# westlake-repl/Adapter4Rec

Measured on NVIDIA B200. Metric: train user-sequences/s (SASRec + BERT-base LoRA r=8 adapter-tuning step: fwd+bwd+allreduce+Adam), higher is better.
Workload: dtype bf16

## Files before the change

adapter4rec_b200/csrc/attention_small.cu:

```cuda
#include "a4r_common.cuh"
#include "mma_sync.cuh"

namespace {

constexpr int LP = 32;
constexpr int WARPS_PER_CTA = 4;

struct AttnParams {
  const __nv_bfloat16* qkv;
  __nv_bfloat16* out;
  const __nv_bfloat16* dout;
  const void* mask;
  int64_t ld_qkv, ld_out, mask_ld;
  int N, L, heads;
  int mask_dtype;
  const int32_t* cu_seqlens;
  int causal;
  float scale, mask_neg;
  uint32_t drop_thr16;
  float drop_scale;
  uint64_t drop_seed, drop_offset;
};

A4R_DEVICE void prob_dropout(float (&s)[2][4][4], const AttnParams& p, int n, int h, int lane) {
  const int g = lane >> 2, t = lane & 3;
  const uint64_t base = p.drop_offset + (static_cast<uint64_t>(n) * p.heads + h) * (32 * 8);
  const uint64_t seed = rng_seed(p.drop_seed);
#pragma unroll
  for (int mt = 0; mt < 2; ++mt)
#pragma unroll
    for (int hh = 0; hh < 2; ++hh) {
      const int i = mt * 16 + hh * 8 + g;
#pragma unroll
      for (int np = 0; np < 2; ++np) {
        const uint64_t r = rng64(seed, base + static_cast<uint64_t>(i) * 8 + np * 4 + t);
#pragma unroll
        for (int q = 0; q < 2; ++q)
#pragma unroll
          for (int e = 0; e < 2; ++e) {
            float& x = s[mt][np * 2 + q][hh * 2 + e];
            x = rng_keep(r, q * 2 + e, p.drop_thr16) ? x * p.drop_scale : 0.0f;
          }
      }
    }
}

template <int COLS>
struct Tile {
  static constexpr int kChunks = COLS / 8;
  static constexpr int kBytes = LP * COLS * 2;
  A4R_DEVICE static uint32_t off(int row, int chunk) {
    const int x = COLS == 64 ? row : (row >> 1);
    return static_cast<uint32_t>(row * COLS * 2 + (((chunk ^ x) & (kChunks - 1)) << 4));
  }
};

template <int COLS>
A4R_DEVICE void load_a(uint32_t (&a)[4], uint32_t base, int m0, int k0, int lane) {
  const int mi = lane >> 3, r = lane & 7;
  const int row = m0 + r + ((mi & 1) << 3);
  const int chunk = (k0 >> 3) + (mi >> 1);
  ldsm_x4(a, base + Tile<COLS>::off(row, chunk));
}
template <int COLS>
A4R_DEVICE void load_a_t(uint32_t (&a)[4], uint32_t base, int m0, int k0, int lane) {
  const int mi = lane >> 3, r = lane & 7;
  const int row = k0 + r + ((mi >> 1) << 3);
  const int chunk = (m0 >> 3) + (mi & 1);
  ldsm_x4_t(a, base + Tile<COLS>::off(row, chunk));
}
template <int COLS>
A4R_DEVICE void load_b_nk(uint32_t (&b)[4], uint32_t base, int n0, int k0, int lane) {
  const int mi = lane >> 3, r = lane & 7;
  const int row = n0 + r + ((mi >> 1) << 3);
  const int chunk = (k0 >> 3) + (mi & 1);
  ldsm_x4(b, base + Tile<COLS>::off(row, chunk));
}
template <int COLS>
A4R_DEVICE void load_b_kn(uint32_t (&b)[4], uint32_t base, int n0, int k0, int lane) {
  const int mi = lane >> 3, r = lane & 7;
  const int row = k0 + r + ((mi & 1) << 3);
  const int chunk = (n0 >> 3) + (mi >> 1);
  ldsm_x4_t(b, base + Tile<COLS>::off(row, chunk));
}

template <int DH>
A4R_DEVICE void load_tile(uint8_t* tile, const __nv_bfloat16* g, int64_t ld, int L, int lane) {
  constexpr int CH = DH / 8;
  const uint32_t base = smem_u32(tile);
#pragma unroll
  for (int i = lane; i < LP * CH; i += 32) {
    const int row = i / CH, ch = i % CH;
    const bool ok = row < L;
    const __nv_bfloat16* src = g + (ok ? static_cast<int64_t>(row) * ld + ch * 8 : 0);
    const int sz = ok ? 16 : 0;
    asm volatile("cp.async.cg.shared.global [%0], [%1], 16, %2;" ::"r"(base + Tile<DH>::off(row, ch)), "l"(src), "r"(sz)
                 : "memory");
// ... 101 lines not shown
#pragma unroll
      for (int nt = 0; nt < 4; ++nt)
#pragma unroll
        for (int e = 0; e < 2; ++e) {
          const float ex = __expf(s[mt][nt][h * 2 + e] - mx);
          s[mt][nt][h * 2 + e] = ex;
          sum += ex;
        }
      sum += __shfl_xor_sync(0xffffffffu, sum, 1);
      sum += __shfl_xor_sync(0xffffffffu, sum, 2);
      const float inv = 1.0f / sum;
#pragma unroll
      for (int nt = 0; nt < 4; ++nt)
#pragma unroll
        for (int e = 0; e < 2; ++e) s[mt][nt][h * 2 + e] *= inv;
    }
  }
}

A4R_DEVICE uint32_t build_keymask(const AttnParams& p, const SeqSpan& sq, int lane) {
  const bool ok = lane < sq.L ? key_valid(p, sq, lane) : false;
  return __ballot_sync(0xffffffffu, ok);
}

A4R_DEVICE void acc_to_a(uint32_t (&a)[4], const float (&c0)[4], const float (&c1)[4]) {
  a[0] = pack_bf16x2(c0[0], c0[1]);
  a[1] = pack_bf16x2(c0[2], c0[3]);
  a[2] = pack_bf16x2(c1[0], c1[1]);
  a[3] = pack_bf16x2(c1[2], c1[3]);
}

template <int DH>
__global__ void __launch_bounds__(WARPS_PER_CTA * 32, 3) attn_fwd_kernel(const AttnParams p) {
  extern __shared__ __align__(128) uint8_t smem_attn[];
  constexpr int TB = Tile<DH>::kBytes;
  const int warp = threadIdx.x >> 5, lane = threadIdx.x & 31;
  uint8_t* my = smem_attn + warp * 3 * TB;
  const int64_t total = static_cast<int64_t>(p.N) * p.heads;
  for (int64_t w = static_cast<int64_t>(blockIdx.x) * WARPS_PER_CTA + warp; w < total;
       w += static_cast<int64_t>(gridDim.x) * WARPS_PER_CTA) {
    const int n = static_cast<int>(w / p.heads), h = static_cast<int>(w % p.heads);
    const int64_t Hd = static_cast<int64_t>(p.heads) * DH;
    const SeqSpan sq = seq_span(p, n);
    const __nv_bfloat16* q = p.qkv + sq.row0 * p.ld_qkv + h * DH;
    load_tile<DH>(my, q, p.ld_qkv, sq.L, lane);
    load_tile<DH>(my + TB, q + Hd, p.ld_qkv, sq.L, lane);
    load_tile<DH>(my + 2 * TB, q + 2 * Hd, p.ld_qkv, sq.L, lane);
    const uint32_t km = build_keymask(p, sq, lane);
    cp_async_wait_all();
    __syncwarp();
    const uint32_t sQ = smem_u32(my), sK = sQ + TB, sV = sK + TB;
    float s[2][4][4];
    scores_softmax<DH>(s, sQ, sK, p, sq.L, lane, km);
    if (p.drop_thr16 != 0) prob_dropout(s, p, n, h, lane);
    float o[2][DH / 8][4];
#pragma unroll
    for (int mt = 0; mt < 2; ++mt)
#pragma unroll
      for (int nt = 0; nt < DH / 8; ++nt)
#pragma unroll
        for (int e = 0; e < 4; ++e) o[mt][nt][e] = 0.0f;
#pragma unroll
    for (int ks = 0; ks < 2; ++ks) {
      uint32_t a0[4], a1[4];
      acc_to_a(a0, s[0][2 * ks], s[0][2 * ks + 1]);
      acc_to_a(a1, s[1][2 * ks], s[1][2 * ks + 1]);
#pragma unroll
      for (int np = 0; np < DH / 16; ++np) {
        uint32_t b[4];
        load_b_kn<DH>(b, sV, np * 16, ks * 16, lane);
        const uint32_t b0[2] = {b[0], b[1]}, b1[2] = {b[2], b[3]};
        mma_bf16_16816(o[0][np * 2], a0, b0);
        mma_bf16_16816(o[0][np * 2 + 1], a0, b1);
        mma_bf16_16816(o[1][np * 2], a1, b0);
        mma_bf16_16816(o[1][np * 2 + 1], a1, b1);
      }
    }
    __syncwarp();
    acc_to_tile<DH, DH / 8>(my, o, 1.f, 1.f, 1.f, 1.f, lane);
    __syncwarp();
    store_tile<DH>(my, p.out + sq.row0 * p.ld_out + h * DH, p.ld_out, sq.L, lane);
    __syncwarp();
  }
}

template <int DH>
__global__ void __launch_bounds__(WARPS_PER_CTA * 32) attn_bwd_kernel(const AttnParams p) {
  extern __shared__ __align__(128) uint8_t smem_attn[];
  constexpr int TB = Tile<DH>::kBytes;
  constexpr int PB = Tile<32>::kBytes;
  const int warp = threadIdx.x >> 5, lane = threadIdx.x & 31;
  uint8_t* my = smem_attn + warp * (4 * TB + 2 * PB);
  const int64_t total = static_cast<int64_t>(p.N) * p.heads;
  for (int64_t w = static_cast<int64_t>(blockIdx.x) * WARPS_PER_CTA + warp; w < total;
       w += static_cast<int64_t>(gridDim.x) * WARPS_PER_CTA) {
    const int n = static_cast<int>(w / p.heads), h = static_cast<int>(w % p.heads);
    const int64_t Hd = static_cast<int64_t>(p.heads) * DH;
    const SeqSpan sq = seq_span(p, n);
    const __nv_bfloat16* q = p.qkv + sq.row0 * p.ld_qkv + h * DH;
    uint8_t *tQ = my, *tK = my + TB, *tV = my + 2 * TB, *tdO = my + 3 * TB, *tP = my + 4 * TB, *tdS = tP + PB;
    load_tile<DH>(tQ, q, p.ld_qkv, sq.L, lane);
    load_tile<DH>(tK, q + Hd, p.ld_qkv, sq.L, lane);
    load_tile<DH>(tV, q + 2 * Hd, p.ld_qkv, sq.L, lane);
    load_tile<DH>(tdO, p.dout + sq.row0 * p.ld_out + h * DH, p.ld_out, sq.L, lane);
    const uint32_t km = build_keymask(p, sq, lane);
    cp_async_wait_all();
    __syncwarp();
    const uint32_t sQ = smem_u32(tQ), sK = smem_u32(tK), sV = smem_u32(tV), sdO = smem_u32(tdO), sP = smem_u32(tP),
                   sdS = smem_u32(tdS);
    float s[2][4][4];
    scores_softmax<DH>(s, sQ, sK, p, sq.L, lane, km);
    float dp[2][4][4];
#pragma unroll
    for (int mt = 0; mt < 2; ++mt)
#pragma unroll
      for (int nt = 0; nt < 4; ++nt)
#pragma unroll
        for (int e = 0; e < 4; ++e) dp[mt][nt][e] = 0.0f;
#pragma unroll
    for (int k0 = 0; k0 < DH; k0 += 16) {
      uint32_t a0[4], a1[4];
      load_a<DH>(a0, sdO, 0, k0, lane);
      load_a<DH>(a1, sdO, 16, k0, lane);
#pragma unroll
      for (int np = 0; np < 2; ++np) {
        uint32_t b[4];
        load_b_nk<DH>(b, sV, np * 16, k0, lane);
        const uint32_t b0[2] = {b[0], b[1]}, b1[2] = {b[2], b[3]};
        mma_bf16_16816(dp[0][np * 2], a0, b0);
        mma_bf16_16816(dp[0][np * 2 + 1], a0, b1);
        mma_bf16_16816(dp[1][np * 2], a1, b0);
        mma_bf16_16816(dp[1][np * 2 + 1], a1, b1);
      }
    }
    float sd[2][4][4];
#pragma unroll
    for (int mt = 0; mt < 2; ++mt)
#pragma unroll
      for (int nt = 0; nt < 4; ++nt)
#pragma unroll
        for (int e = 0; e < 4; ++e) sd[mt][nt][e] = s[mt][nt][e];
    if (p.drop_thr16 != 0) {
      prob_dropout(sd, p, n, h, lane);
#pragma unroll
      for (int mt = 0; mt < 2; ++mt)
#pragma unroll
        for (int nt = 0; nt < 4; ++nt)
#pragma unroll
          for (int e = 0; e < 4; ++e) dp[mt][nt][e] = (sd[mt][nt][e] != 0.0f) ? dp[mt][nt][e] * p.drop_scale : 0.0f;
    }
#pragma unroll
    for (int mt = 0; mt < 2; ++mt)
#pragma unroll
      for (int hh = 0; hh < 2; ++hh) {
        float d = 0.0f;
#pragma unroll
        for (int nt = 0; nt < 4; ++nt)
#pragma unroll
          for (int e = 0; e < 2; ++e) d += s[mt][nt][hh * 2 + e] * dp[mt][nt][hh * 2 + e];
        d += __shfl_xor_sync(0xffffffffu, d, 1);
        d += __shfl_xor_sync(0xffffffffu, d, 2);
#pragma unroll
        for (int nt = 0; nt < 4; ++nt)
#pragma unroll
          for (int e = 0; e < 2; ++e)
            dp[mt][nt][hh * 2 + e] = s[mt][nt][hh * 2 + e] * (dp[mt][nt][hh * 2 + e] - d) * p.scale;
      }
    acc_to_tile<32, 4>(tP, sd, 1.f, 1.f, 1.f, 1.f, lane);
    acc_to_tile<32, 4>(tdS, dp, 1.f, 1.f, 1.f, 1.f, lane);
    __syncwarp();
    float acc[2][DH / 8][4];
#pragma unroll
    for (int mt = 0; mt < 2; ++mt)
#pragma unroll
      for (int nt = 0; nt < DH / 8; ++nt)
#pragma unroll
        for (int e = 0; e < 4; ++e) acc[mt][nt][e] = 0.0f;
#pragma unroll
    for (int ks = 0; ks < 2; ++ks) {
      uint32_t a0[4], a1[4];
      acc_to_a(a0, dp[0][2 * ks], dp[0][2 * ks + 1]);
      acc_to_a(a1, dp[1][2 * ks], dp[1][2 * ks + 1]);
#pragma unroll
      for (int np = 0; np < DH / 16; ++np) {
        uint32_t b[4];
        load_b_kn<DH>(b, sK, np * 16, ks * 16, lane);
        const uint32_t b0[2] = {b[0], b[1]}, b1[2] = {b[2], b[3]};
        mma_bf16_16816(acc[0][np * 2], a0, b0);
        mma_bf16_16816(acc[0][np * 2 + 1], a0, b1);
        mma_bf16_16816(acc[1][np * 2], a1, b0);
        mma_bf16_16816(acc[1][np * 2 + 1], a1, b1);
      }
    }
    float dk[2][DH / 8][4], dv[2][DH / 8][4];
#pragma unroll
    for (int mt = 0; mt < 2; ++mt)
#pragma unroll
      for (int nt = 0; nt < DH / 8; ++nt)
#pragma unroll
        for (int e = 0; e < 4; ++e) dk[mt][nt][e] = dv[mt][nt][e] = 0.0f;
#pragma unroll
    for (int ks = 0; ks < 2; ++ks) {
      uint32_t a0[4], a1[4], p0[4], p1[4];
      load_a_t<32>(a0, sdS, 0, ks * 16, lane);
      load_a_t<32>(a1, sdS, 16, ks * 16, lane);
      load_a_t<32>(p0, sP, 0, ks * 16, lane);
      load_a_t<32>(p1, sP, 16, ks * 16, lane);
#pragma unroll
      for (int np = 0; np < DH / 16; ++np) {
        uint32_t b[4];
        load_b_kn<DH>(b, sQ, np * 16, ks * 16, lane);
        const uint32_t b0[2] = {b[0], b[1]}, b1[2] = {b[2], b[3]};
        mma_bf16_16816(dk[0][np * 2], a0, b0);
        mma_bf16_16816(dk[0][np * 2 + 1], a0, b1);
        mma_bf16_16816(dk[1][np * 2], a1, b0);
        mma_bf16_16816(dk[1][np * 2 + 1], a1, b1);
        uint32_t c[4];
        load_b_kn<DH>(c, sdO, np * 16, ks * 16, lane);
        const uint32_t c0[2] = {c[0], c[1]}, c1[2] = {c[2], c[3]};
        mma_bf16_16816(dv[0][np * 2], p0, c0);
        mma_bf16_16816(dv[0][np * 2 + 1], p0, c1);
        mma_bf16_16816(dv[1][np * 2], p1, c0);
        mma_bf16_16816(dv[1][np * 2 + 1], p1, c1);
      }
    }
    __syncwarp();
    acc_to_tile<DH, DH / 8>(tQ, acc, 1.f, 1.f, 1.f, 1.f, lane);
    acc_to_tile<DH, DH / 8>(tK, dk, 1.f, 1.f, 1.f, 1.f, lane);
    acc_to_tile<DH, DH / 8>(tV, dv, 1.f, 1.f, 1.f, 1.f, lane);
    __syncwarp();
    __nv_bfloat16* dq = p.out + sq.row0 * p.ld_qkv + h * DH;
    store_tile<DH>(tQ, dq, p.ld_qkv, sq.L, lane);
    store_tile<DH>(tK, dq + Hd, p.ld_qkv, sq.L, lane);
    store_tile<DH>(tV, dq + 2 * Hd, p.ld_qkv, sq.L, lane);
    __syncwarp();
  }
}

int check_common(const a4r_attn_args* a) {
  A4R_CHECK_ARG(a != nullptr, "attention: args is NULL");
  A4R_CHECK_ARG(a->qkv && a->out, "attention: qkv/out must be non-NULL");
  A4R_CHECK_ARG(a->L >= 1 && a->L <= LP, "attention_small: L must be in [1,32] (got %lld)", (long long)a->L);
  A4R_CHECK_ARG(a->head_dim == 32 || a->head_dim == 64, "attention_small: head_dim must be 32 or 64");
  A4R_CHECK_ARG(a->heads >= 1 && a->N >= 0, "attention: bad heads/N");
  A4R_CHECK_ARG(a->ld_qkv >= 3 * a->heads * a->head_dim && a->ld_qkv % 8 == 0, "attention: bad ld_qkv");
  A4R_CHECK_ARG(a->ld_out >= a->heads * a->head_dim && a->ld_out % 8 == 0, "attention: bad ld_out");
  A4R_CHECK_ARG(a4r_aligned16(a->qkv) && a4r_aligned16(a->out), "attention: pointers must be 16B aligned");
  A4R_CHECK_ARG(a->mask_dtype >= 0 && a->mask_dtype <= 2, "attention: mask_dtype must be 0,1,2");
  if (a->mask_dtype != 0)
    A4R_CHECK_ARG(a->mask != nullptr && (a->cu_seqlens != nullptr || a->mask_ld >= a->L), "attention: bad mask/mask_ld");
  A4R_CHECK_ARG(a->dropout_p >= 0.0f && a->dropout_p < 1.0f, "attention: dropout_p must be in [0,1)");
  return a4r_device_check();
}

AttnParams to_params(const a4r_attn_args* a) {
  AttnParams p;
  p.qkv = static_cast<const __nv_bfloat16*>(a->qkv);
  p.out = static_cast<__nv_bfloat16*>(a->out);
  p.dout = static_cast<const __nv_bfloat16*>(a->dout);
  p.mask = a->mask;
  p.ld_qkv = a->ld_qkv;
  p.ld_out = a->ld_out;
  p.mask_ld = a->mask_ld;
  p.N = static_cast<int>(a->N);
  p.L = static_cast<int>(a->L);
  p.cu_seqlens = a->cu_seqlens;
  p.heads = static_cast<int>(a->heads);
  p.mask_dtype = a->mask_dtype;
  p.causal = a->causal;
  p.scale = a->scale;
  p.mask_neg = a->mask_neg;
  p.drop_thr16 = static_cast<uint32_t>(a->dropout_p * 65536.0f + 0.5f);
  p.drop_scale = 65536.0f / static_cast<float>(65536u - p.drop_thr16);
  p.drop_seed = a->dropout_seed;
  p.drop_offset = a->dropout_offset;
  return p;
}

template <typename K>
int launch(K kernel, int smem, const AttnParams& p, cudaStream_t stream, bool* attr_done) {
  if (!*attr_done) {
    A4R_CUDA_OK(cudaFuncSetAttribute(kernel, cudaFuncAttributeMaxDynamicSharedMemorySize, smem));
    *attr_done = true;
  }
  const int64_t total = static_cast<int64_t>(p.N) * p.heads;
  int64_t blocks = (total + WARPS_PER_CTA - 1) / WARPS_PER_CTA;
  const int64_t cap = static_cast<int64_t>(a4r_num_sms()) * 8;
  if (blocks > cap) blocks = cap;
  kernel<<<static_cast<int>(blocks), WARPS_PER_CTA * 32, smem, stream>>>(p);
  A4R_LAUNCH_OK();
  a4r_count_launch(1);
  return A4R_OK;
}

}

extern "C" int a4r_attn_small_fwd(const a4r_attn_args* a, a4r_stream_t stream) {
  int rc = check_common(a);
  if (rc != A4R_OK) return rc;
  if (a->N == 0) return A4R_OK;
  const AttnParams p = to_params(a);
  static bool done64 = false, done32 = false;
  if (a->head_dim == 64)
    return launch(attn_fwd_kernel<64>, WARPS_PER_CTA * 3 * Tile<64>::kBytes, p, static_cast<cudaStream_t>(stream), &done64);
  return launch(attn_fwd_kernel<32>, WARPS_PER_CTA * 3 * Tile<32>::kBytes, p, static_cast<cudaStream_t>(stream), &done32);
}

extern "C" int a4r_attn_small_bwd(const a4r_attn_args* a, a4r_stream_t stream) {
  int rc = check_common(a);
  if (rc != A4R_OK) return rc;
  A4R_CHECK_ARG(a->dout != nullptr && a4r_aligned16(a->dout), "attention bwd: dout missing or unaligned");
  if (a->N == 0) return A4R_OK;
  const AttnParams p = to_params(a);
  static bool done64 = false, done32 = false;
  if (a->head_dim == 64)
    return launch(attn_bwd_kernel<64>, WARPS_PER_CTA * (4 * Tile<64>::kBytes + 2 * Tile<32>::kBytes), p,
                  static_cast<cudaStream_t>(stream), &done64);
  return launch(attn_bwd_kernel<32>, WARPS_PER_CTA * (4 * Tile<32>::kBytes + 2 * Tile<32>::kBytes), p,
                static_cast<cudaStream_t>(stream), &done32);
}
```

adapter4rec_b200/functional.py:

```python
import torch

from . import ops

BF16 = torch.bfloat16


PARAM_EPOCH = [0]


def bump_param_epoch():
    PARAM_EPOCH[0] += 1


class WeightCache:

    def __init__(self):
        self.key = None
        self.master = None
        self.w = None
        self.wt = None

    def get(self, weight, need_t=False):
        key = (weight.data_ptr(), weight._version, weight.device, PARAM_EPOCH[0] if weight.requires_grad else -1)
        if key != self.key:
# ... 230 lines not shown
        if cls.seed_address is not None:
            return cls.SEED_INDIRECT | int(cls.seed_address), off
        return cls.seed, off

    @classmethod
    def replay_seed(cls, step, base=None):
        z = ((cls.seed if base is None else int(base)) + 0x9E3779B97F4A7C15 * (int(step) + 1)) & 0xFFFFFFFFFFFFFFFF
        z = ((z ^ (z >> 30)) * 0xBF58476D1CE4E5B9) & 0xFFFFFFFFFFFFFFFF
        z = ((z ^ (z >> 27)) * 0x94D049BB133111EB) & 0xFFFFFFFFFFFFFFFF
        return (z ^ (z >> 31)) & 0x7FFFFFFFFFFFFFFF


class DropoutAddFunction(torch.autograd.Function):

    @staticmethod
    def forward(ctx, x, res, p):
        ctx.p = p
        ctx.rng = DropoutState.draw((x.numel() + 3) // 4)
        ctx.has_res = res is not None
        return ops.dropout(x.contiguous(), None if res is None else res.contiguous(), p, *ctx.rng)

    @staticmethod
    def backward(ctx, dy):
        dy = dy.contiguous()
        dx = ops.dropout(dy, None, ctx.p, *ctx.rng) if ctx.needs_input_grad[0] else None
        return dx, (dy if ctx.has_res and ctx.needs_input_grad[1] else None), None


def dropout_add(x, res, p):
    return DropoutAddFunction.apply(x, res, float(p))


class AddFunction(torch.autograd.Function):

    @staticmethod
    def forward(ctx, x, res):
        return ops.dropout(x.contiguous(), res.contiguous(), 0.0, 0, 0)

    @staticmethod
    def backward(ctx, dy):
        return (dy if ctx.needs_input_grad[0] else None), (dy if ctx.needs_input_grad[1] else None)


def add(x, res):
    return AddFunction.apply(x, res)


class AttentionFunction(torch.autograd.Function):
    @staticmethod
    def forward(ctx, qkv, mask, N, L, heads, head_dim, causal, mask_neg, dropout_p=0.0, scale=None, cu_seqlens=None):
        ctx.cfg = (N, L, heads, head_dim, causal, mask_neg, scale)
        ctx.cu = cu_seqlens
        ctx.mask = mask
        ctx.drop = None
        if dropout_p > 0.0:
            ctx.drop = (dropout_p,) + DropoutState.draw(N * heads * 32 * 8)
        out, lse = ops.attn_small_fwd(qkv, N, L, heads, head_dim, mask=mask, causal=causal, mask_neg=mask_neg, want_lse=True,
                                      dropout=ctx.drop, scale=scale, cu_seqlens=cu_seqlens)
        ctx.save_for_backward(qkv, lse, out if lse is not None else None)
        return out

    @staticmethod
    def backward(ctx, dctx):
        qkv, lse, out = ctx.saved_tensors
        N, L, heads, head_dim, causal, mask_neg, scale = ctx.cfg
        dqkv = ops.attn_small_bwd(qkv, dctx.contiguous(), N, L, heads, head_dim, mask=ctx.mask, causal=causal,
                                  mask_neg=mask_neg, lse=lse, ctx=out, dropout=ctx.drop, scale=scale, cu_seqlens=ctx.cu)
        return dqkv, None, None, None, None, None, None, None, None, None, None


def attention(qkv, mask, N, L, heads, head_dim, causal=False, mask_neg=ops.F32_MIN, dropout_p=0.0, scale=None,
              cu_seqlens=None):
    return AttentionFunction.apply(qkv, mask, N, L, heads, head_dim, causal, mask_neg, float(dropout_p), scale, cu_seqlens)


class GatherRowsFunction(torch.autograd.Function):

    @staticmethod
    def forward(ctx, x, idx):
        ctx.rows = x.shape[0]
        ctx.save_for_backward(idx)
        return ops.gather_rows(x.contiguous(), idx)

    @staticmethod
    def backward(ctx, dy):
        (idx,) = ctx.saved_tensors
        dx = torch.zeros((ctx.rows, dy.shape[1]), dtype=dy.dtype, device=dy.device)
        dx.index_copy_(0, idx, dy.contiguous())
        return dx, None


def gather_rows(x, idx):
    return GatherRowsFunction.apply(x, idx)


class ExpandRowsFunction(torch.autograd.Function):

    @staticmethod
    def forward(ctx, x, inverse, counts):
        ctx.save_for_backward(inverse, counts)
        return ops.gather_rows(x.contiguous(), inverse)

    @staticmethod
    def backward(ctx, dy):
        inverse, counts = ctx.saved_tensors
        order = torch.argsort(inverse, stable=True)
        grouped = dy.contiguous()[order].float()
        return torch.segment_reduce(grouped, "sum", lengths=counts, axis=0).to(dy.dtype), None, None


def expand_rows(x, inverse, counts):
    return ExpandRowsFunction.apply(x, inverse, counts)


_ROW_HASH = {}


def unique_rows(rows):
    N, W = rows.shape
    key = (rows.device, W)
# ... 404 lines not shown
```

adapter4rec_b200/lib.py:

```python
import ctypes
import os
from ctypes import POINTER, Structure, c_char_p, c_float, c_int32, c_int64, c_size_t, c_void_p

HERE = os.path.dirname(os.path.abspath(__file__))
LIB_PATH = os.path.join(HERE, "libadapter4rec_sm100.so")

A4R_OK, A4R_EINVAL, A4R_ECUDA, A4R_EARCH, A4R_EWORKSPACE = 0, -1, -2, -3, -4
EPI_LINEAR, EPI_GELU, EPI_RELU, EPI_DGELU, EPI_DRELU = 0, 1, 2, 3, 4


class GemmArgs(Structure):
    _fields_ = [
        ("A", c_void_p), ("lda", c_int64), ("B", c_void_p), ("ldb", c_int64),
        ("A2", c_void_p), ("lda2", c_int64), ("B2", c_void_p), ("ldb2", c_int64), ("K2", c_int64),
        ("C", c_void_p), ("ldc", c_int64), ("aux", c_void_p), ("ldaux", c_int64),
        ("residual", c_void_p), ("ldr", c_int64), ("residual2", c_void_p), ("ldr2", c_int64),
        ("bias", c_void_p), ("M", c_int64), ("N", c_int64), ("K", c_int64),
        ("alpha", c_float), ("epilogue", c_int32), ("out_f32", c_int32), ("block_n", c_int32),
        ("dropout_p", c_float), ("dropout_seed", ctypes.c_uint64), ("dropout_offset", ctypes.c_uint64),
        ("dropout_after_residual", c_int32),
    ]


class AttnArgs(Structure):
    _fields_ = [
        ("qkv", c_void_p), ("out", c_void_p), ("dout", c_void_p), ("mask", c_void_p),
        ("ld_qkv", c_int64), ("ld_out", c_int64), ("mask_ld", c_int64),
        ("N", c_int64), ("L", c_int64), ("heads", c_int64), ("head_dim", c_int64),
        ("mask_dtype", c_int32), ("causal", c_int32), ("scale", c_float), ("mask_neg", c_float),
        ("lse", c_void_p), ("ctx", c_void_p),
        ("dropout_p", c_float), ("dropout_seed", ctypes.c_uint64), ("dropout_offset", ctypes.c_uint64),
        ("cu_seqlens", c_void_p),
    ]


class EmbedArgs(Structure):
    _fields_ = [
        ("ids", c_void_p), ("ld_ids", c_int64), ("word_emb", c_void_p), ("pos_emb", c_void_p),
        ("type_emb", c_void_p), ("prompt", c_void_p), ("gamma", c_void_p), ("beta", c_void_p),
        ("out", c_void_p), ("z_out", c_void_p), ("mean_out", c_void_p), ("rstd_out", c_void_p),
        ("N", c_int64), ("L", c_int64), ("H", c_int64), ("pos_offset", c_int64),
        ("roberta_pad_id", c_int64), ("n_prompt", c_int64), ("eps", c_float),
    ]


class BceArgs(Structure):
    _fields_ = [
        ("prec", c_void_p), ("emb", c_void_p), ("log_mask", c_void_p), ("pos_score", c_void_p),
        ("neg_score", c_void_p), ("loss", c_void_p), ("count", c_void_p),
        ("B", c_int64), ("S", c_int64), ("D", c_int64), ("cpc", c_int32),
    ]


class AdapterArgs(Structure):
    _fields_ = [
        ("h", c_void_p), ("ldh", c_int64), ("input", c_void_p), ("ldi", c_int64),
        ("w_down", c_void_p), ("b_down", c_void_p), ("w_up", c_void_p), ("b_up", c_void_p),
        ("gamma", c_void_p), ("beta", c_void_p), ("out", c_void_p), ("z_out", c_void_p),
        ("mean", c_void_p), ("rstd", c_void_p), ("s_out", c_void_p), ("u_out", c_void_p),
        ("M", c_int64), ("H", c_int64), ("r", c_int64), ("act", c_int32), ("tail", c_int32), ("eps", c_float),
        ("lds", c_int64), ("impl", c_int32),
    ]


class InbatchCeArgs(Structure):
    _fields_ = [
        ("prec", c_void_p), ("cand", c_void_p), ("ld_cand", c_int64), ("item_ids", c_void_p), ("log_mask", c_void_p),
        ("cand_bias", c_void_p), ("lse", c_void_p), ("loss", c_void_p), ("count", c_void_p),
        ("B", c_int64), ("S", c_int64), ("D", c_int64), ("masked_logit", c_float),
    ]


PROTOTYPES = {
    "a4r_version": (c_int32, []),
    "a4r_last_error_string": (c_char_p, []),
    "a4r_device_check": (c_int32, []),
    "a4r_launch_count": (c_int64, []),
    "a4r_gemm_bf16_tn": (c_int32, [POINTER(GemmArgs), c_void_p]),
    "a4r_attn_small_fwd": (c_int32, [POINTER(AttnArgs), c_void_p]),
    "a4r_attn_small_bwd": (c_int32, [POINTER(AttnArgs), c_void_p]),
    "a4r_attn_mid_fwd": (c_int32, [POINTER(AttnArgs), c_void_p]),
    "a4r_attn_mid_bwd": (c_int32, [POINTER(AttnArgs), c_void_p]),
    "a4r_layernorm_fwd": (c_int32, [c_void_p, c_void_p, c_int64, c_void_p, c_void_p, c_float, c_void_p, c_void_p,
                                    c_void_p, c_void_p, c_int64, c_int64, c_void_p]),
    "a4r_layernorm_bwd_workspace_bytes": (c_size_t, [c_int64]),
# ... 72 lines not shown
```

adapter4rec_b200/ops.py:

```python
import ctypes

import torch

from . import lib as _l
from .lib import EPI_DGELU, EPI_DRELU, EPI_GELU, EPI_LINEAR, EPI_RELU

BF16 = torch.bfloat16
F32_MIN = -3.4028234663852886e38


def _stream():
    return ctypes.c_void_p(torch.cuda.current_stream().cuda_stream)


def _p(t):
    return None if t is None else ctypes.c_void_p(t.data_ptr())


def _rows2d(t, name):
    if t.dim() != 2 or t.stride(1) != 1:
        raise ValueError("%s must be 2-D with unit column stride, got shape %s stride %s" % (name, tuple(t.shape), t.stride()))
    return t.stride(0) if t.shape[0] > 1 else max(t.stride(0), t.shape[1])


# ... 71 lines not shown
    assert out.dtype in (BF16, torch.float32)
    if _gemm_profile is not None:
        e0, e1 = torch.cuda.Event(enable_timing=True), torch.cuda.Event(enable_timing=True)
        e0.record()
        _l.check(_l.get_lib().a4r_gemm_bf16_tn(ctypes.byref(g), _stream()), "a4r_gemm_bf16_tn")
        e1.record()
        k2 = a2.shape[1] if a2 is not None else 0
        _gemm_profile.append((2.0 * M * N * (K + k2), e0, e1, (M, N, K + k2, int(epilogue))))
        return out
    _l.check(_l.get_lib().a4r_gemm_bf16_tn(ctypes.byref(g), _stream()), "a4r_gemm_bf16_tn")
    return out


def dropout(x, res, p, seed, offset):
    assert x.dtype == BF16 and x.is_contiguous() and (res is None or (res.dtype == BF16 and res.is_contiguous() and res.shape == x.shape))
    out = torch.empty_like(x)
    _l.check(_l.get_lib().a4r_dropout(_p(x), _p(res), _p(out), x.numel(), float(p), int(seed), int(offset), _stream()),
             "a4r_dropout")
    return out


def _attn_args(qkv, N, L, heads, head_dim, mask, causal, mask_neg, dropout=None, scale=None, cu_seqlens=None):
    a = _l.AttnArgs()
    if cu_seqlens is not None:
        assert cu_seqlens.dtype == torch.int32 and cu_seqlens.is_contiguous() and cu_seqlens.numel() == N + 1 and L <= 32
        a.cu_seqlens = _p(cu_seqlens)
        if mask is not None:
            assert mask.dim() == 1 and mask.numel() == qkv.shape[0] and mask.is_contiguous()
            a.mask, a.mask_ld = _p(mask), 0
            a.mask_dtype = {torch.int64: 1, torch.float32: 2}[mask.dtype]
    if dropout is not None:
        a.dropout_p, a.dropout_seed, a.dropout_offset = float(dropout[0]), int(dropout[1]), int(dropout[2])
    a.qkv, a.ld_qkv = _p(qkv), _rows2d(qkv, "qkv")
    a.N, a.L, a.heads, a.head_dim = N, L, heads, head_dim
    if mask is None:
        a.mask_dtype = 0
    elif cu_seqlens is None:
        assert mask.dim() == 2 and mask.shape[0] == N and mask.shape[1] >= L and mask.stride(1) == 1
        a.mask, a.mask_ld = _p(mask), mask.stride(0)
        a.mask_dtype = {torch.int64: 1, torch.float32: 2}[mask.dtype]
    a.causal, a.scale, a.mask_neg = int(causal), (float(head_dim) ** -0.5 if scale is None else float(scale)), float(mask_neg)
    return a


def _attn_kernel(L, head_dim, causal, direction):
    lib = _l.get_lib()
    if L <= 32:
        return (lib.a4r_attn_small_fwd if direction == "fwd" else lib.a4r_attn_small_bwd), "a4r_attn_small_" + direction
    if L <= 256 and head_dim == 64 and not causal:
        return (lib.a4r_attn_mid_fwd if direction == "fwd" else lib.a4r_attn_mid_bwd), "a4r_attn_mid_" + direction
    raise RuntimeError("attention: unsupported shape L=%d head_dim=%d causal=%s (no fallback exists)" % (L, head_dim, causal))


def attn_small_fwd(qkv, N, L, heads, head_dim, mask=None, causal=False, mask_neg=F32_MIN, want_lse=False, dropout=None,
                   scale=None, cu_seqlens=None):
    assert qkv.dtype == BF16 and (cu_seqlens is not None or qkv.shape[0] == N * L)
    out = torch.empty((qkv.shape[0], heads * head_dim), dtype=BF16, device=qkv.device)
    a = _attn_args(qkv, N, L, heads, head_dim, mask, causal, mask_neg, dropout, scale, cu_seqlens)
    a.out, a.ld_out = _p(out), out.stride(0)
    lse = None
    if want_lse and L > 32:
        lse = torch.empty((N * L, heads), dtype=torch.float32, device=qkv.device)
        a.lse = _p(lse)
    fn, name = _attn_kernel(L, head_dim, causal, "fwd")
    _l.check(fn(ctypes.byref(a), _stream()), name)
    return (out, lse) if want_lse else out


def attn_small_bwd(qkv, dctx, N, L, heads, head_dim, mask=None, causal=False, mask_neg=F32_MIN, lse=None, ctx=None,
                   dropout=None, scale=None, cu_seqlens=None):
    assert qkv.dtype == BF16 and dctx.dtype == BF16 and dctx.shape[0] == qkv.shape[0]
    assert cu_seqlens is not None or qkv.shape[0] == N * L
    dqkv = torch.empty((qkv.shape[0], 3 * heads * head_dim), dtype=BF16, device=qkv.device)
    a = _attn_args(qkv, N, L, heads, head_dim, mask, causal, mask_neg, dropout, scale, cu_seqlens)
    assert _rows2d(qkv, "qkv") == dqkv.stride(0), "attention bwd expects a contiguous qkv"
    a.out, a.dout, a.ld_out = _p(dqkv), _p(dctx), _rows2d(dctx, "dctx")
    if L > 32:
        assert lse is not None and ctx is not None and ctx.is_contiguous() and dctx.is_contiguous()
        a.lse, a.ctx = _p(lse), _p(ctx)
    fn, name = _attn_kernel(L, head_dim, causal, "bwd")
    _l.check(fn(ctypes.byref(a), _stream()), name)
    return dqkv


def layernorm_fwd(x, gamma, beta, eps, res=None, want_z=False, want_stats=True):
    assert x.dtype == BF16 and x.is_contiguous() and x.dim() == 2
    M, H = x.shape
    y = torch.empty_like(x)
    z = torch.empty_like(x) if want_z else None
    mean = torch.empty(M, dtype=torch.float32, device=x.device) if want_stats else None
    rstd = torch.empty(M, dtype=torch.float32, device=x.device) if want_stats else None
    res_rows = 0
    if res is not None:
        assert res.dtype == BF16 and res.is_contiguous() and res.shape[-1] == H
        res_rows = res.numel() // H
    _l.check(_l.get_lib().a4r_layernorm_fwd(_p(x), _p(res), res_rows, _p(gamma), _p(beta), float(eps), _p(y), _p(z),
                                            _p(mean), _p(rstd), M, H, _stream()), "a4r_layernorm_fwd")
    return y, z, mean, rstd


def layernorm_bwd(dy, z, mean, rstd, gamma, dgamma=None, dbeta=None, accumulate=False, masked=None):
    assert dy.dtype == BF16 and z.dtype == BF16 and dy.is_contiguous() and z.is_contiguous()
    M, H = z.shape
    dz = torch.empty_like(z)
    dzm = torch.empty_like(z) if masked is not None else None
    mp, mseed, moff = masked if masked is not None else (0.0, 0, 0)
    ws, wsb = None, 0
    if dgamma is not None:
        wsb = _l.get_lib().a4r_layernorm_bwd_workspace_bytes(H)
        ws = workspace(wsb, z.device)
    _l.check(_l.get_lib().a4r_layernorm_bwd(_p(dy), _p(z), _p(mean), _p(rstd), _p(gamma), _p(dz), _p(dgamma), _p(dbeta),
                                            int(accumulate), _p(ws), wsb, M, H, _p(dzm), float(mp), int(mseed), int(moff),
                                            _stream()), "a4r_layernorm_bwd")
    return (dz, dzm) if masked is not None else dz


def layernorm_bwd_add(dy, z, mean, rstd, gamma, dskip):
    assert dy.dtype == BF16 and z.dtype == BF16 and dskip.dtype == BF16
    assert dy.is_contiguous() and z.is_contiguous() and dskip.is_contiguous() and dskip.shape == z.shape
    M, H = z.shape
    dz = torch.empty_like(z)
    _l.check(_l.get_lib().a4r_layernorm_bwd_add(_p(dy), _p(z), _p(mean), _p(rstd), _p(gamma), _p(dskip), _p(dz), M, H,
                                                _stream()), "a4r_layernorm_bwd_add")
    return dz


def embed_ln_fwd(ids, L, word_emb, pos_emb, type_emb, gamma, beta, eps, pos_offset=0, roberta_pad_id=-1, prompt=None,
                 want_z=False):
    assert ids.dtype == torch.int64 and ids.dim() == 2 and ids.stride(1) == 1
# ... 338 lines not shown
```

include/adapter4rec.h:

```cpp
#ifndef ADAPTER4REC_H_
#define ADAPTER4REC_H_

#include <stddef.h>
#include <stdint.h>

#ifdef __cplusplus
extern "C" {
#endif

#define A4R_OK 0
#define A4R_EINVAL (-1)
#define A4R_ECUDA (-2)
#define A4R_EARCH (-3)
#define A4R_EWORKSPACE (-4)

typedef void* a4r_stream_t;

#define A4R_API __attribute__((visibility("default")))

A4R_API int a4r_version(void);
A4R_API const char* a4r_last_error_string(void);
A4R_API int a4r_device_check(void);
A4R_API int64_t a4r_launch_count(void);

// ... 4 lines not shown
  A4R_EPI_DGELU = 3,
  A4R_EPI_DRELU = 4
};

typedef struct a4r_gemm_args {
  const void* A;
  int64_t lda;
  const void* B;
  int64_t ldb;
  const void* A2;
  int64_t lda2;
  const void* B2;
  int64_t ldb2;
  int64_t K2;
  void* C;
  int64_t ldc;
  void* aux;
  int64_t ldaux;
  const void* residual;
  int64_t ldr;
  const void* residual2;
  int64_t ldr2;
  const float* bias;
  int64_t M, N, K;
  float alpha;
  int32_t epilogue;
  int32_t out_f32;
  int32_t block_n;
  float dropout_p;
  uint64_t dropout_seed;
  uint64_t dropout_offset;
  int32_t dropout_after_residual;
} a4r_gemm_args;

A4R_API int a4r_gemm_bf16_tn(const a4r_gemm_args* args, a4r_stream_t stream);

typedef struct a4r_attn_args {
  const void* qkv;
  void* out;
  const void* dout;
  const void* mask;
  int64_t ld_qkv, ld_out, mask_ld;
  int64_t N, L, heads, head_dim;
  int32_t mask_dtype;
  int32_t causal;
  float scale;
  float mask_neg;
  float* lse;
  const void* ctx;
  float dropout_p;
  uint64_t dropout_seed;
  uint64_t dropout_offset;
  const int32_t* cu_seqlens;
} a4r_attn_args;

A4R_API int a4r_attn_small_fwd(const a4r_attn_args* args, a4r_stream_t stream);
A4R_API int a4r_attn_small_bwd(const a4r_attn_args* args, a4r_stream_t stream);

A4R_API int a4r_attn_mid_fwd(const a4r_attn_args* args, a4r_stream_t stream);
A4R_API int a4r_attn_mid_bwd(const a4r_attn_args* args, a4r_stream_t stream);

A4R_API int a4r_layernorm_fwd(const void* x, const void* res, int64_t res_rows, const float* gamma, const float* beta,
                      float eps, void* y, void* z_out, float* mean, float* rstd, int64_t M, int64_t H,
                      a4r_stream_t stream);
A4R_API size_t a4r_layernorm_bwd_workspace_bytes(int64_t H);
A4R_API int a4r_layernorm_bwd(const void* dy, const void* z, const float* mean, const float* rstd, const float* gamma,
                      void* dz, float* dgamma, float* dbeta, int32_t accumulate, void* workspace,
                      size_t workspace_bytes, int64_t M, int64_t H, void* dz_masked, float dropout_p,
                      uint64_t dropout_seed, uint64_t dropout_offset, a4r_stream_t stream);
A4R_API int a4r_layernorm_bwd_add(const void* dy, const void* z, const float* mean, const float* rstd, const float* gamma,
                          const void* dskip, void* dz, int64_t M, int64_t H, a4r_stream_t stream);

typedef struct a4r_adapter_args {
  const void* h;
  int64_t ldh;
  const void* input;
  int64_t ldi;
  const void* w_down;
  const float* b_down;
  const void* w_up;
  const float* b_up;
  const float* gamma;
  const float* beta;
  void* out;
  void* z_out;
  float* mean;
  float* rstd;
  void* s_out;
  void* u_out;
  int64_t M, H, r;
  int32_t act;
  int32_t tail;
  float eps;
  int64_t lds;
  int32_t impl;
} a4r_adapter_args;
A4R_API int a4r_adapter_ln_supported(int64_t H, int64_t r);
A4R_API int a4r_adapter_ln_fwd(const a4r_adapter_args* args, a4r_stream_t stream);

typedef struct a4r_embed_args {
  const int64_t* ids;
  int64_t ld_ids;
  const void* word_emb;
  const void* pos_emb;
  const void* type_emb;
  const void* prompt;
// ... 105 lines not shown
```

Baseline: 1966.

## Cache attention dropout keep-mask bits from forward for reuse in backward

The forward small-attention kernel now packs the per-element dropout keep decisions into one 32-bit row mask per lane and writes them to a buffer. The backward kernel reads those bits and applies them instead of regenerating the random numbers, which removes RNG work from the backward pass. The backward also splits the dQ/dK/dV accumulation into separate scoped blocks, each stored immediately, to lower register pressure. The cost is an extra small global buffer plus shuffle work to pack and unpack the bits.

```diff
diff --git a/adapter4rec_b200/csrc/attention_small.cu b/adapter4rec_b200/csrc/attention_small.cu
--- a/adapter4rec_b200/csrc/attention_small.cu
+++ b/adapter4rec_b200/csrc/attention_small.cu
@@ -20,9 +20,11 @@
   uint32_t drop_thr16;
   float drop_scale;
   uint64_t drop_seed, drop_offset;
+  uint32_t* drop_bits;
 };
 
-A4R_DEVICE void prob_dropout(float (&s)[2][4][4], const AttnParams& p, int n, int h, int lane) {
+
+A4R_DEVICE void prob_dropout(float (&s)[2][4][4], const AttnParams& p, int n, int h, int lane, uint32_t (&u)[4]) {
   const int g = lane >> 2, t = lane & 3;
   const uint64_t base = p.drop_offset + (static_cast<uint64_t>(n) * p.heads + h) * (32 * 8);
   const uint64_t seed = rng_seed(p.drop_seed);
@@ -31,6 +33,7 @@
 #pragma unroll
     for (int hh = 0; hh < 2; ++hh) {
       const int i = mt * 16 + hh * 8 + g;
+      uint32_t v = 0;
 #pragma unroll
       for (int np = 0; np < 2; ++np) {
         const uint64_t r = rng64(seed, base + static_cast<uint64_t>(i) * 8 + np * 4 + t);
@@ -39,10 +42,50 @@
 #pragma unroll
           for (int e = 0; e < 2; ++e) {
             float& x = s[mt][np * 2 + q][hh * 2 + e];
-            x = rng_keep(r, q * 2 + e, p.drop_thr16) ? x * p.drop_scale : 0.0f;
+            const bool keep = rng_keep(r, q * 2 + e, p.drop_thr16);
+            x = keep ? x * p.drop_scale : 0.0f;
+            if (keep) v |= 1u << ((np * 2 + q) * 8 + e);
           }
       }
-    }
+      u[mt * 2 + hh] = v;
+    }
+}
+
+A4R_DEVICE void apply_keep(float (&s)[2][4][4], const uint32_t (&u)[4], float scale) {
+#pragma unroll
+  for (int mt = 0; mt < 2; ++mt)
+#pragma unroll
+    for (int nt = 0; nt < 4; ++nt)
+#pragma unroll
+      for (int hh = 0; hh < 2; ++hh)
+#pragma unroll
+        for (int e = 0; e < 2; ++e) {
+          float& x = s[mt][nt][hh * 2 + e];
+          x = ((u[mt * 2 + hh] >> (nt * 8 + e)) & 1u) ? x * scale : 0.0f;
+        }
+}
+
+A4R_DEVICE uint32_t keep_to_row(const uint32_t (&u)[4], int lane) {
+  uint32_t w[4];
+#pragma unroll
+  for (int r4 = 0; r4 < 4; ++r4) {
+    uint32_t v = u[r4] << (2 * (lane & 3));
+    v |= __shfl_xor_sync(0xffffffffu, v, 1);
+    v |= __shfl_xor_sync(0xffffffffu, v, 2);
+    w[r4] = v;
+  }
+  uint32_t row = 0;
+#pragma unroll
+  for (int r4 = 0; r4 < 4; ++r4) {
+    const uint32_t v = __shfl_sync(0xffffffffu, w[r4], (lane & 7) * 4);
+    if ((lane >> 3) == r4) row = v;
+  }
+  return row;
+}
+
+A4R_DEVICE void row_to_keep(uint32_t row, int lane, uint32_t (&u)[4]) {
+#pragma unroll
+  for (int r4 = 0; r4 < 4; ++r4) u[r4] = (__shfl_sync(0xffffffffu, row, r4 * 8 + (lane >> 2)) >> (2 * (lane & 3))) & 0x03030303u;
 }
 
 template <int COLS>
@@ -250,7 +293,11 @@
     const uint32_t sQ = smem_u32(my), sK = sQ + TB, sV = sK + TB;
     float s[2][4][4];
     scores_softmax<DH>(s, sQ, sK, p, sq.L, lane, km);
-    if (p.drop_thr16 != 0) prob_dropout(s, p, n, h, lane);
+    if (p.drop_thr16 != 0) {
+      uint32_t u[4];
+      prob_dropout(s, p, n, h, lane, u);
+      if (p.drop_bits != nullptr) p.drop_bits[w * 32 + lane] = keep_to_row(u, lane);
+    }
     float o[2][DH / 8][4];
 #pragma unroll
     for (int mt = 0; mt < 2; ++mt)
@@ -302,6 +349,7 @@
     load_tile<DH>(tV, q + 2 * Hd, p.ld_qkv, sq.L, lane);
     load_tile<DH>(tdO, p.dout + sq.row0 * p.ld_out + h * DH, p.ld_out, sq.L, lane);
     const uint32_t km = build_keymask(p, sq, lane);
+    const uint32_t keep_row = p.drop_thr16 != 0 && p.drop_bits != nullptr ? p.drop_bits[w * 32 + lane] : 0u;
     cp_async_wait_all();
     __syncwarp();
     const uint32_t sQ = smem_u32(tQ), sK = smem_u32(tK), sV = smem_u32(tV), sdO = smem_u32(tdO), sP = smem_u32(tP),
@@ -339,7 +387,13 @@
 #pragma unroll
         for (int e = 0; e < 4; ++e) sd[mt][nt][e] = s[mt][nt][e];
     if (p.drop_thr16 != 0) {
-      prob_dropout(sd, p, n, h, lane);
+      uint32_t u[4];
+      if (p.drop_bits != nullptr) {
+        row_to_keep(keep_row, lane, u);
+        apply_keep(sd, u, p.drop_scale);
+      } else {
+        prob_dropout(sd, p, n, h, lane, u);
+      }
 #pragma unroll
       for (int mt = 0; mt < 2; ++mt)
 #pragma unroll
@@ -367,70 +421,93 @@
     acc_to_tile<32, 4>(tP, sd, 1.f, 1.f, 1.f, 1.f, lane);
     acc_to_tile<32, 4>(tdS, dp, 1.f, 1.f, 1.f, 1.f, lane);
     __syncwarp();
-    float acc[2][DH / 8][4];
-#pragma unroll
-    for (int mt = 0; mt < 2; ++mt)
-#pragma unroll
-      for (int nt = 0; nt < DH / 8; ++nt)
-#pragma unroll
-        for (int e = 0; e < 4; ++e) acc[mt][nt][e] = 0.0f;
-#pragma unroll
-    for (int ks = 0; ks < 2; ++ks) {
-      uint32_t a0[4], a1[4];
-      acc_to_a(a0, dp[0][2 * ks], dp[0][2 * ks + 1]);
-      acc_to_a(a1, dp[1][2 * ks], dp[1][2 * ks + 1]);
-#pragma unroll
-      for (int np = 0; np < DH / 16; ++np) {
-        uint32_t b[4];
-        load_b_kn<DH>(b, sK, np * 16, ks * 16, lane);
-        const uint32_t b0[2] = {b[0], b[1]}, b1[2] = {b[2], b[3]};
-        mma_bf16_16816(acc[0][np * 2], a0, b0);
-        mma_bf16_16816(acc[0][np * 2 + 1], a0, b1);
-        mma_bf16_16816(acc[1][np * 2], a1, b0);
-        mma_bf16_16816(acc[1][np * 2 + 1], a1, b1);
-      }
-    }
-    float dk[2][DH / 8][4], dv[2][DH / 8][4];
-#pragma unroll
-    for (int mt = 0; mt < 2; ++mt)
-#pragma unroll
-      for (int nt = 0; nt < DH / 8; ++nt)
-#pragma unroll
-        for (int e = 0; e < 4; ++e) dk[mt][nt][e] = dv[mt][nt][e] = 0.0f;
-#pragma unroll
-    for (int ks = 0; ks < 2; ++ks) {
-      uint32_t a0[4], a1[4], p0[4], p1[4];
-      load_a_t<32>(a0, sdS, 0, ks * 16, lane);
-      load_a_t<32>(a1, sdS, 16, ks * 16, lane);
-      load_a_t<32>(p0, sP, 0, ks * 16, lane);
-      load_a_t<32>(p1, sP, 16, ks * 16, lane);
-#pragma unroll
-      for (int np = 0; np < DH / 16; ++np) {
-        uint32_t b[4];
-        load_b_kn<DH>(b, sQ, np * 16, ks * 16, lane);
-        const uint32_t b0[2] = {b[0], b[1]}, b1[2] = {b[2], b[3]};
-        mma_bf16_16816(dk[0][np * 2], a0, b0);
-        mma_bf16_16816(dk[0][np * 2 + 1], a0, b1);
-        mma_bf16_16816(dk[1][np * 2], a1, b0);
-        mma_bf16_16816(dk[1][np * 2 + 1], a1, b1);
-        uint32_t c[4];
-        load_b_kn<DH>(c, sdO, np * 16, ks * 16, lane);
-        const uint32_t c0[2] = {c[0], c[1]}, c1[2] = {c[2], c[3]};
-        mma_bf16_16816(dv[0][np * 2], p0, c0);
-        mma_bf16_16816(dv[0][np * 2 + 1], p0, c1);
-        mma_bf16_16816(dv[1][np * 2], p1, c0);
-        mma_bf16_16816(dv[1][np * 2 + 1], p1, c1);
-      }
-    }
-    __syncwarp();
-    acc_to_tile<DH, DH / 8>(tQ, acc, 1.f, 1.f, 1.f, 1.f, lane);
-    acc_to_tile<DH, DH / 8>(tK, dk, 1.f, 1.f, 1.f, 1.f, lane);
-    acc_to_tile<DH, DH / 8>(tV, dv, 1.f, 1.f, 1.f, 1.f, lane);
-    __syncwarp();
     __nv_bfloat16* dq = p.out + sq.row0 * p.ld_qkv + h * DH;
-    store_tile<DH>(tQ, dq, p.ld_qkv, sq.L, lane);
-    store_tile<DH>(tK, dq + Hd, p.ld_qkv, sq.L, lane);
-    store_tile<DH>(tV, dq + 2 * Hd, p.ld_qkv, sq.L, lane);
+    {
+      float acc[2][DH / 8][4];
+#pragma unroll
+      for (int mt = 0; mt < 2; ++mt)
+#pragma unroll
+        for (int nt = 0; nt < DH / 8; ++nt)
+#pragma unroll
+          for (int e = 0; e < 4; ++e) acc[mt][nt][e] = 0.0f;
+#pragma unroll
+      for (int ks = 0; ks < 2; ++ks) {
+        uint32_t a0[4], a1[4];
+        acc_to_a(a0, dp[0][2 * ks], dp[0][2 * ks + 1]);
+        acc_to_a(a1, dp[1][2 * ks], dp[1][2 * ks + 1]);
+#pragma unroll
+        for (int np = 0; np < DH / 16; ++np) {
+          uint32_t b[4];
+          load_b_kn<DH>(b, sK, np * 16, ks * 16, lane);
+          const uint32_t b0[2] = {b[0], b[1]}, b1[2] = {b[2], b[3]};
+          mma_bf16_16816(acc[0][np * 2], a0, b0);
+          mma_bf16_16816(acc[0][np * 2 + 1], a0, b1);
+          mma_bf16_16816(acc[1][np * 2], a1, b0);
+          mma_bf16_16816(acc[1][np * 2 + 1], a1, b1);
+        }
+      }
+      acc_to_tile<DH, DH / 8>(tV, acc, 1.f, 1.f, 1.f, 1.f, lane);
+      __syncwarp();
+      store_tile<DH>(tV, dq, p.ld_qkv, sq.L, lane);
+    }
+    {
+      float dk[2][DH / 8][4];
+#pragma unroll
+      for (int mt = 0; mt < 2; ++mt)
+#pragma unroll
+        for (int nt = 0; nt < DH / 8; ++nt)
+#pragma unroll
+          for (int e = 0; e < 4; ++e) dk[mt][nt][e] = 0.0f;
+#pragma unroll
+      for (int ks = 0; ks < 2; ++ks) {
+        uint32_t a0[4], a1[4];
+        load_a_t<32>(a0, sdS, 0, ks * 16, lane);
+        load_a_t<32>(a1, sdS, 16, ks * 16, lane);
+#pragma unroll
+        for (int np = 0; np < DH / 16; ++np) {
+          uint32_t b[4];
+          load_b_kn<DH>(b, sQ, np * 16, ks * 16, lane);
+          const uint32_t b0[2] = {b[0], b[1]}, b1[2] = {b[2], b[3]};
+          mma_bf16_16816(dk[0][np * 2], a0, b0);
+          mma_bf16_16816(dk[0][np * 2 + 1], a0, b1);
+          mma_bf16_16816(dk[1][np * 2], a1, b0);
+          mma_bf16_16816(dk[1][np * 2 + 1], a1, b1);
+        }
+      }
+      __syncwarp();
+      acc_to_tile<DH, DH / 8>(tK, dk, 1.f, 1.f, 1.f, 1.f, lane);
+      __syncwarp();
+      store_tile<DH>(tK, dq + Hd, p.ld_qkv, sq.L, lane);
+    }
+    {
+      float dv[2][DH / 8][4];
+#pragma unroll
+      for (int mt = 0; mt < 2; ++mt)
+#pragma unroll
+        for (int nt = 0; nt < DH / 8; ++nt)
+#pragma unroll
+          for (int e = 0; e < 4; ++e) dv[mt][nt][e] = 0.0f;
+#pragma unroll
+      for (int ks = 0; ks < 2; ++ks) {
+        uint32_t p0[4], p1[4];
+        load_a_t<32>(p0, sP, 0, ks * 16, lane);
+        load_a_t<32>(p1, sP, 16, ks * 16, lane);
+#pragma unroll
+        for (int np = 0; np < DH / 16; ++np) {
+          uint32_t c[4];
+          load_b_kn<DH>(c, sdO, np * 16, ks * 16, lane);
+          const uint32_t c0[2] = {c[0], c[1]}, c1[2] = {c[2], c[3]};
+          mma_bf16_16816(dv[0][np * 2], p0, c0);
+          mma_bf16_16816(dv[0][np * 2 + 1], p0, c1);
+          mma_bf16_16816(dv[1][np * 2], p1, c0);
+          mma_bf16_16816(dv[1][np * 2 + 1], p1, c1);
+        }
+      }
+      __syncwarp();
+      acc_to_tile<DH, DH / 8>(tQ, dv, 1.f, 1.f, 1.f, 1.f, lane);
+      __syncwarp();
+      store_tile<DH>(tQ, dq + 2 * Hd, p.ld_qkv, sq.L, lane);
+    }
     __syncwarp();
   }
 }
@@ -448,6 +525,7 @@
   if (a->mask_dtype != 0)
     A4R_CHECK_ARG(a->mask != nullptr && (a->cu_seqlens != nullptr || a->mask_ld >= a->L), "attention: bad mask/mask_ld");
   A4R_CHECK_ARG(a->dropout_p >= 0.0f && a->dropout_p < 1.0f, "attention: dropout_p must be in [0,1)");
+  A4R_CHECK_ARG(reinterpret_cast<uintptr_t>(a->dropout_bits) % 4 == 0, "attention: dropout_bits must be 4B aligned");
   return a4r_device_check();
 }
 
@@ -472,6 +550,7 @@
   p.drop_scale = 65536.0f / static_cast<float>(65536u - p.drop_thr16);
   p.drop_seed = a->dropout_seed;
   p.drop_offset = a->dropout_offset;
+  p.drop_bits = a->dropout_bits;
   return p;
 }
 
diff --git a/adapter4rec_b200/functional.py b/adapter4rec_b200/functional.py
--- a/adapter4rec_b200/functional.py
+++ b/adapter4rec_b200/functional.py
@@ -306,11 +306,13 @@
         ctx.cfg = (N, L, heads, head_dim, causal, mask_neg, scale)
         ctx.cu = cu_seqlens
         ctx.mask = mask
-        ctx.drop = None
+        ctx.drop = ctx.bits = None
         if dropout_p > 0.0:
             ctx.drop = (dropout_p,) + DropoutState.draw(N * heads * 32 * 8)
+            if L <= 32:
+                ctx.bits = torch.empty(N * heads * 32, dtype=torch.int32, device=qkv.device)
         out, lse = ops.attn_small_fwd(qkv, N, L, heads, head_dim, mask=mask, causal=causal, mask_neg=mask_neg, want_lse=True,
-                                      dropout=ctx.drop, scale=scale, cu_seqlens=cu_seqlens)
+                                      dropout=ctx.drop, scale=scale, cu_seqlens=cu_seqlens, drop_bits=ctx.bits)
         ctx.save_for_backward(qkv, lse, out if lse is not None else None)
         return out
 
@@ -319,7 +321,8 @@
         qkv, lse, out = ctx.saved_tensors
         N, L, heads, head_dim, causal, mask_neg, scale = ctx.cfg
         dqkv = ops.attn_small_bwd(qkv, dctx.contiguous(), N, L, heads, head_dim, mask=ctx.mask, causal=causal,
-                                  mask_neg=mask_neg, lse=lse, ctx=out, dropout=ctx.drop, scale=scale, cu_seqlens=ctx.cu)
+                                  mask_neg=mask_neg, lse=lse, ctx=out, dropout=ctx.drop, scale=scale, cu_seqlens=ctx.cu,
+                                  drop_bits=ctx.bits)
         return dqkv, None, None, None, None, None, None, None, None, None, None
 
 
diff --git a/adapter4rec_b200/lib.py b/adapter4rec_b200/lib.py
--- a/adapter4rec_b200/lib.py
+++ b/adapter4rec_b200/lib.py
@@ -30,7 +30,7 @@
         ("mask_dtype", c_int32), ("causal", c_int32), ("scale", c_float), ("mask_neg", c_float),
         ("lse", c_void_p), ("ctx", c_void_p),
         ("dropout_p", c_float), ("dropout_seed", ctypes.c_uint64), ("dropout_offset", ctypes.c_uint64),
-        ("cu_seqlens", c_void_p),
+        ("cu_seqlens", c_void_p), ("dropout_bits", c_void_p),
     ]
 
 
diff --git a/adapter4rec_b200/ops.py b/adapter4rec_b200/ops.py
--- a/adapter4rec_b200/ops.py
+++ b/adapter4rec_b200/ops.py
@@ -147,12 +147,19 @@
     raise RuntimeError("attention: unsupported shape L=%d head_dim=%d causal=%s (no fallback exists)" % (L, head_dim, causal))
 
 
+def _drop_bits_arg(a, drop_bits, N, heads, L):
+    if drop_bits is not None:
+        assert L <= 32 and drop_bits.dtype == torch.int32 and drop_bits.is_contiguous() and drop_bits.numel() == N * heads * 32
+        a.dropout_bits = _p(drop_bits)
+
+
 def attn_small_fwd(qkv, N, L, heads, head_dim, mask=None, causal=False, mask_neg=F32_MIN, want_lse=False, dropout=None,
-                   scale=None, cu_seqlens=None):
+                   scale=None, cu_seqlens=None, drop_bits=None):
     assert qkv.dtype == BF16 and (cu_seqlens is not None or qkv.shape[0] == N * L)
     out = torch.empty((qkv.shape[0], heads * head_dim), dtype=BF16, device=qkv.device)
     a = _attn_args(qkv, N, L, heads, head_dim, mask, causal, mask_neg, dropout, scale, cu_seqlens)
     a.out, a.ld_out = _p(out), out.stride(0)
+    _drop_bits_arg(a, drop_bits, N, heads, L)
     lse = None
     if want_lse and L > 32:
         lse = torch.empty((N * L, heads), dtype=torch.float32, device=qkv.device)
@@ -163,13 +170,14 @@
 
 
 def attn_small_bwd(qkv, dctx, N, L, heads, head_dim, mask=None, causal=False, mask_neg=F32_MIN, lse=None, ctx=None,
-                   dropout=None, scale=None, cu_seqlens=None):
+                   dropout=None, scale=None, cu_seqlens=None, drop_bits=None):
     assert qkv.dtype == BF16 and dctx.dtype == BF16 and dctx.shape[0] == qkv.shape[0]
     assert cu_seqlens is not None or qkv.shape[0] == N * L
     dqkv = torch.empty((qkv.shape[0], 3 * heads * head_dim), dtype=BF16, device=qkv.device)
     a = _attn_args(qkv, N, L, heads, head_dim, mask, causal, mask_neg, dropout, scale, cu_seqlens)
     assert _rows2d(qkv, "qkv") == dqkv.stride(0), "attention bwd expects a contiguous qkv"
     a.out, a.dout, a.ld_out = _p(dqkv), _p(dctx), _rows2d(dctx, "dctx")
+    _drop_bits_arg(a, drop_bits, N, heads, L)
     if L > 32:
         assert lse is not None and ctx is not None and ctx.is_contiguous() and dctx.is_contiguous()
         a.lse, a.ctx = _p(lse), _p(ctx)
diff --git a/include/adapter4rec.h b/include/adapter4rec.h
--- a/include/adapter4rec.h
+++ b/include/adapter4rec.h
@@ -80,6 +80,7 @@
   uint64_t dropout_seed;
   uint64_t dropout_offset;
   const int32_t* cu_seqlens;
+  uint32_t* dropout_bits;
 } a4r_attn_args;
 
 A4R_API int a4r_attn_small_fwd(const a4r_attn_args* args, a4r_stream_t stream);
```

Result: faster. 1988 (median of 6 runs) (+1.1%).
